# kutieme/avenir

Measured on AMD Instinct MI355X. Metric: naive_bayes_train_rows_per_s, higher is better.
Workload: dtype row-packed categorical records (11-bit records, lossless)/int64 counts (exact); 1 GPU; model=NaiveBayes(resource/churn.json: 5 categorical features, 2 classes), global_batch=1073741824, rows_per_gpu=1073741824, parallelism=dp1

## Files before the change

avenir_amd/csrc/bindings.cpp:

```cpp
#include <algorithm>
#include <atomic>
#include <cstdlib>
#include <condition_variable>
#include <cstring>
#include <functional>
#include <chrono>
#include <limits>
#include <map>
#include <memory>
#include <mutex>
#include <thread>
#include <unistd.h>
#include <sys/stat.h>
#include <sys/mman.h>
#include <fcntl.h>
#include <torch/extension.h>
#include <ATen/hip/impl/HIPGuardImplMasqueradingAsCUDA.h>
#include <ATen/hip/impl/HIPStreamMasqueradingAsCUDA.h>

#include "avenir_kernels.h"
#include "avenir_host.h"

namespace {

// ... 200 lines not shown
                  reinterpret_cast<uint32_t*>(dense.data_ptr<int>()), cur_stream(words));
  return dense;
}

void class_histogram_radix(const at::Tensor& dense, int64_t n, int64_t B, std::vector<int64_t> radices,
                           std::vector<int64_t> bins_host, std::vector<int64_t> offs_host, int64_t class_radix,
                           int64_t total_bins, int64_t n_classes, at::Tensor& out, bool count_labels) {
  CHECK_DEV(dense);
  CHECK_DTYPE(dense, at::kInt);
  TORCH_CHECK(B >= 4 && B <= 15 && n >= 0 && dense.numel() >= avk::dense_words(n, (int)B), "radix stream too short");
  const int64_t F = (int64_t)radices.size();
  TORCH_CHECK(F >= 1 && F <= 8, "1..8 packed fields");
  const auto rad = radix_ints(radices, F, "radices"), hb = radix_ints(bins_host, F, "bins");
  const auto ho = radix_ints(offs_host, F, "offs");
  TORCH_CHECK(n_classes >= 1 && n_classes <= 2, "1 or 2 classes");
  TORCH_CHECK(total_bins >= 1 && total_bins < (int64_t(1) << 24), "bad table width");
  CHECK_DEV(out); CHECK_DTYPE(out, at::kLong);
  TORCH_CHECK(out.numel() == n_classes * total_bins, "out must be [C * TB]");
  DevGuard g(dense.device());
  avk::class_histogram_radix(reinterpret_cast<const uint32_t*>(dense.data_ptr<int>()), n, (int)B, rad.data(), hb.data(),
                             ho.data(), (int)F, (int)class_radix, (int)total_bins, (int)n_classes,
                             count_labels ? 1 : 0, reinterpret_cast<unsigned long long*>(out.data_ptr<int64_t>()),
                             cur_stream(dense));
}

int64_t radix_recip(int64_t d) {
  TORCH_CHECK(d >= 1 && d <= (int64_t(1) << 15), "divisor out of range");
  return (int64_t)avk::radix_recip((unsigned)d);
}

void pair_histogram(const at::Tensor& codes, int64_t n, const c10::optional<at::Tensor>& labels,
                    const at::Tensor& bins, const at::Tensor& pairs, const at::Tensor& poff,
                    int64_t max_tab, int64_t n_classes, at::Tensor& out) {
  CHECK_DEV(codes);
  CHECK_DTYPE(codes, at::kByte);
  TORCH_CHECK(codes.dim() == 2 && n <= codes.size(1), "codes must be [F, ld>=n]");
  CHECK_DEV(bins);
  CHECK_DTYPE(bins, at::kInt);
  CHECK_DEV(pairs);
  CHECK_DTYPE(pairs, at::kInt);
  CHECK_DEV(poff);
  CHECK_DTYPE(poff, at::kLong);
  CHECK_DEV(out);
  CHECK_DTYPE(out, at::kLong);
  TORCH_CHECK(pairs.dim() == 2 && pairs.size(1) == 2, "pairs must be [P,2]");
  TORCH_CHECK(poff.numel() == pairs.size(0), "poff must be [P]");
// ... 4108 lines not shown
  avk::lstm_bwd(dhseq.data_ptr<float>(), reinterpret_cast<const unsigned short*>(gates.data_ptr()),
                cseq.data_ptr<float>(), ptr_or_null<float>(c0), ptr_or_null<float>(dhn), ptr_or_null<float>(dcn),
                wfragT.data_ptr(), (int)B, (int)T, (int)H, (int)KS, RT,
                reinterpret_cast<unsigned short*>(dz.data_ptr()), dh0.data_ptr<float>(), dc0.data_ptr<float>(),
                cur_stream(dhseq));
  return {dz, dh0, dc0};
}

}

void register_comm(py::module_& m);

PYBIND11_MODULE(_C, m) {
  register_comm(m);
  m.doc() = "avenir_amd native kernels (HIP/CDNA4 gfx950) and host runtime";
  m.def("class_histogram", &class_histogram);
  m.def("pair_histogram", &pair_histogram);
  m.def("class_histogram_rowpacked", &class_histogram_rowpacked);
  m.def("pack_dense", &pack_dense);
  m.def("class_histogram_dense", &class_histogram_dense);
  m.def("radix_shape", &radix_shape);
  m.def("pack_radix", &pack_radix);
  m.def("class_histogram_radix", &class_histogram_radix);
  m.def("radix_recip", &radix_recip);
  m.def("bigram_histogram", &bigram_histogram);
  m.def("class_moments", &class_moments);
  m.def("nb_predict", &nb_predict);
  m.def("nb_predict_wide", &nb_predict_wide);
  m.def("node_histogram", &node_histogram, py::arg("codes"), py::arg("n"), py::arg("labels"), py::arg("node"),
        py::arg("weight"), py::arg("bins"), py::arg("offs"), py::arg("total_bins"), py::arg("n_classes"),
        py::arg("n_nodes"), py::arg("hist"), py::arg("node_rows") = py::none());
  m.def("node_grad_histogram", &node_grad_histogram, py::arg("codes"), py::arg("n"), py::arg("node"), py::arg("g"),
        py::arg("h"), py::arg("bins"), py::arg("offs"), py::arg("total_bins"), py::arg("n_nodes"), py::arg("out"),
        py::arg("even_only") = false, py::arg("tot_slot") = -1, py::arg("scale") = 65536.0);
  m.def("gbt_grad", &gbt_grad);
  m.def("gbt_split", &gbt_split);
  m.def("rank_avg", &rank_avg);
  m.def("tfidf_csr", &tfidf_csr);
  m.def("mixed_knn", &mixed_knn);
  m.def("pagerank", &pagerank);
  m.def("pagerank_multi", &pagerank_multi);
  m.def("sgns_hot_replicas", &avk::sgns_hot_replicas);
  m.def("sgns_step", &sgns_step, py::arg("Win"), py::arg("Wout"), py::arg("gIn"), py::arg("gOut"), py::arg("cIn"),
        py::arg("cOut"), py::arg("centre"), py::arg("context"), py::arg("aprob"), py::arg("alias"), py::arg("neg"),
        py::arg("lr"), py::arg("mean_in"), py::arg("seed"), py::arg("step"), py::arg("hot") = py::none(),
        py::arg("gOutHot") = py::none(), py::arg("gInHot") = py::none(), py::arg("cIn_next") = py::none(),
// ... 248 lines not shown
```

avenir_amd/csrc/include/avenir_kernels.h:

```cpp
#pragma once
#include <hip/hip_runtime.h>
#include <stdint.h>
#include <algorithm>
#include <stdexcept>

namespace avk {

void class_histogram(const uint8_t* codes, long long ld, long long n, const uint8_t* labels,
                     const int* d_bins, const int* d_offs, const int* h_bins, int nfeat,
                     int total_bins, int n_classes, int count_labels, unsigned long long* out,
                     int mode, hipStream_t stream);
void class_histogram_wide(const uint16_t* codes, long long ld, long long n, const uint8_t* labels, const int* d_bins,
                          const int* d_offs, int nfeat, int total_bins, int n_classes, int count_labels,
                          unsigned long long* out, int mode, hipStream_t stream);
void class_histogram_i32(const int* codes, long long ld, long long n, const uint8_t* labels, const int* d_bins,
                          const int* d_offs, int nfeat, int total_bins, int n_classes, int count_labels,
                          unsigned long long* out, int mode, hipStream_t stream);
void pair_histogram(const uint8_t* codes, long long ld, long long n, const uint8_t* labels,
                    const int* d_bins, const int* d_pairs, const long long* d_poff, int n_pairs,
                    int max_tab, int n_classes, unsigned long long* out, hipStream_t stream);
void bigram_histogram(const int16_t* states, long long n, int L, const uint8_t* labels,
                      int n_classes, int S, unsigned long long* out, hipStream_t stream);
void class_moments(const float* x, long long ld, long long n, int nfeat, const uint8_t* labels,
                   int n_classes, double* part, int nblocks, double* out, hipStream_t stream);
// ... 297 lines not shown
void linear_act_bwd(const float* dY, const float* Y, float* dZ, float* partial, int M, int N, int act,
                    hipStream_t stream);
int linear_act_wgrad_slices(int M, int N, int K);
void linear_act_wgrad(const float* dY, const float* Y, const float* X, float* dZ, float* pW, float* tmp, float* out,
                      int M, int N, int K, int act, hipStream_t stream);
long long forest_predict_bin_lds(int n_nodes, int nfeat);
void forest_predict_bin(const uint8_t* codes, long long ld, long long n, int nfeat, const uint2* nodes, int n_nodes,
                        const float* values, int V, const int* tree_root, const float* tree_w, int n_trees, int mode,
                        float* out, hipStream_t stream);
long long dense_words(long long n, int B);
void pack_dense(const uint16_t* words, long long n, int B, uint32_t* dense, hipStream_t stream);
void class_histogram_dense(const uint32_t* dense, long long n, int B, const int* h_shift, const int* h_width,
                           int nfeat, int label_shift, int label_width, const int* d_bins, const int* d_offs,
                           int total_bins, int n_classes, int count_labels, unsigned long long* out,
                           hipStream_t stream);
int radix_bits(long long J);
int radix_replicas(long long J, int n_classes, int total_bins);
void pack_radix(const uint16_t* words, long long n, int B, const int* h_shift, const int* h_width, const int* h_radix,
                const int* h_bins, int nfeat, int label_shift, int class_radix, int n_classes, uint32_t* dense,
                hipStream_t stream);
void class_histogram_radix(const uint32_t* dense, long long n, int B, const int* h_radix, const int* h_bins,
                           const int* h_offs, int nfeat, int class_radix, int total_bins, int n_classes,
                           int count_labels, unsigned long long* out, hipStream_t stream);
unsigned radix_recip(unsigned d);
long long csv_chunks(long long size);
unsigned long long csv_slow_tokens_take(hipStream_t stream);
unsigned long long rec_slow_tokens_take(hipStream_t stream);
void csv_newline_counts(const uint8_t* bytes, long long size, unsigned* counts, hipStream_t stream);
void csv_newline_positions(const uint8_t* bytes, long long size, const long long* offsets, long long* pos,
                           hipStream_t stream);
void csv_line_bounds(const uint8_t* bytes, const long long* pos, long long nl, long long* starts, long long* ends,
                     uint8_t* keep, unsigned long long* blank, hipStream_t stream);
void csv_parse_rows(const uint8_t* bytes, long long size_padded, const long long* starts, const long long* ends,
                    long long n, char delim, const void* specs, int nspecs, int max_ord, const int* tabs,
                    const int* voff, const int* vlen, const uint8_t* vbytes, int ntab, int nvoc, int nvb,
                    unsigned long long* short_rows, hipStream_t stream);
int csv_devspec_bytes();
void resample_uniform(unsigned long long seed, unsigned long long stream, long long base, long long n, float* out,
                      hipStream_t st);
void smote(const float* X, const float* Xn, const int* nn, const int* Cs, const int* Cn, long long m, int k, int D,
           int Dc, int mult, long long gbase, unsigned long long seed, int exponential, float exp_mean, float* outX,
           int* outC, int* outPick, hipStream_t st);
void gbt_grad(const float* F, int K, int k, const uint8_t* y, long long n, long long row_off, unsigned long long seed,
              unsigned rate32, float* g, float* h, double* loss, hipStream_t stream);
void gbt_split(const long long* hist, const long long* parent, const long long* left, long long* out_hist, int A,
               int TB, int tot, const int* pfeat, const int* pthr, const int* pstart, const int* pend,
// ... 132 lines not shown
```

avenir_amd/csrc/kernels/histogram.hip:

```cpp
#include <cstdlib>
#include <string>

#include "avenir_common.h"
#include "avenir_kernels.h"

namespace {

constexpr int HB = 256;
constexpr int FLUSH_EVERY = 15;

__device__ __forceinline__ void flush_packed(unsigned long long& lo, unsigned long long& hi,
                                             unsigned int* s_bins ) {
  const unsigned long long M = 0x00FF00FF00FF00FFull;
  unsigned long long w[4] = {lo & M, (lo >> 8) & M, hi & M, (hi >> 8) & M};
#pragma unroll
  for (int q = 0; q < 4; ++q) w[q] = av::wave_sum_u64(w[q]);
  if (av::lane_id() == 0) {
#pragma unroll
    for (int q = 0; q < 4; ++q) {
      const int base = (q >> 1) * 8 + (q & 1);
#pragma unroll
      for (int k = 0; k < 4; ++k) {
        unsigned v = (unsigned)((w[q] >> (16 * k)) & 0xFFFFu);
        if (v) atomicAdd(&s_bins[base + 2 * k], v);
// ... 636 lines not shown
      const int bit = k * B, i = bit >> 5, sh = bit & 31;
#pragma unroll
      for (int q = 0; q < 16; ++q) {
        if (q == i) d[q] |= v << sh;
        if (q == i + 1 && sh + B > 32) d[q] |= v >> (32 - sh);
      }
    }
    for (int i = 0; i < B; ++i) dense[g * B + i] = d[i];
  }
}

struct RadixSpec {
  int rad[8];
  int bins[8];
  int offs[8];
  int crad;
  unsigned stride[8], srcp[8], rrcp[8], crcp;
};

__device__ __forceinline__ unsigned div_small(unsigned n, unsigned d, unsigned m) {
  return d == 1u ? n : __umulhi(n, m);
}

__global__ __launch_bounds__(HB) void pack_radix_kernel(const uint16_t* __restrict__ words, long long n, int B,
                                                        RowPackSpec spec, RadixSpec rs, int nfeat,
                                                        uint32_t* __restrict__ dense) {
  const long long groups = (n + 31) >> 5;
  const long long stride = (long long)gridDim.x * HB;
  for (long long g = (long long)blockIdx.x * HB + threadIdx.x; g < groups; g += stride) {
    uint32_t d[16];
#pragma unroll
    for (int i = 0; i < 16; ++i) d[i] = 0;
    for (int k = 0; k < 32; ++k) {
      const long long r = (g << 5) + k;
      uint32_t v = 0;
      if (r < n) {
        const uint32_t w = words[r];
        uint32_t mult = 1;
        if (rs.crad > 1) {
          const uint32_t lb = __builtin_amdgcn_ubfe(w, (unsigned)spec.lsh, 2u);
          const uint32_t cd = lb == 1u ? 0u : (lb == 2u ? 1u : 2u);
          v = min(cd, (uint32_t)rs.crad - 1u);
          mult = (uint32_t)rs.crad;
        }
        for (int f = 0; f < nfeat; ++f) {
          const uint32_t code = __builtin_amdgcn_ubfe(w, (unsigned)spec.sh[f], (unsigned)spec.w[f]);
          v += min(code, (uint32_t)rs.rad[f] - 1u) * mult;
          mult *= (uint32_t)rs.rad[f];
        }
      }
      const int bit = k * B, i = bit >> 5, sh = bit & 31;
#pragma unroll
      for (int q = 0; q < 16; ++q) {
        if (q == i) d[q] |= v << sh;
        if (q == i + 1 && sh + B > 32) d[q] |= v >> (32 - sh);
      }
    }
    for (int i = 0; i < B; ++i) dense[g * B + i] = d[i];
  }
}

template <int B>
__global__ __launch_bounds__(1024) void hist_joint_radix_kernel(const uint32_t* __restrict__ dense, long long n,
                                                                RadixSpec rs, int J, int log2r, int nfeat,
                                                                int n_classes, int total_bins, int count_labels,
                                                                unsigned long long* __restrict__ out) {
  extern __shared__ __attribute__((aligned(16))) unsigned int s_joint[];
  constexpr unsigned M = (1u << B) - 1u;
  const int NT = (int)blockDim.x;
  const int R = 1 << log2r;
  const int ctb = n_classes * total_bins;
  unsigned int* s_small = s_joint + ((size_t)J << log2r);
  const long long groups = (n + 31) >> 5;
  const long long stride = (long long)gridDim.x * NT;
  uint32_t d[B + 1];
  d[B] = 0;
  auto load = [&](long long g) __attribute__((always_inline)) {
    const uint32_t* src = dense + g * B;
#pragma unroll
    for (int i = 0; i < B; ++i) d[i] = src[i];
  };
  long long g = (long long)blockIdx.x * NT + threadIdx.x;
  if (g < groups) load(g);
  for (int i = threadIdx.x; i < (J << log2r) + ctb; i += NT) s_joint[i] = 0;
  char* const my = reinterpret_cast<char*>(s_joint + (threadIdx.x & (unsigned)(R - 1)));
  const unsigned lr = (unsigned)log2r + 2u;
  __syncthreads();
  while (g < groups) {
    const long long left = n - (g << 5);
    auto rec = [&](int k) __attribute__((always_inline)) -> unsigned {
      const int bit = k * B, i = bit >> 5, sh = bit & 31;
      if (sh + B <= 32) return __builtin_amdgcn_ubfe(d[i], (unsigned)sh, (unsigned)B);
      return __builtin_amdgcn_alignbit(d[i + 1], d[i], (unsigned)sh) & M;
    };
    if (left >= 32) {
#pragma unroll
      for (int k = 0; k < 32; ++k) atomicAdd(reinterpret_cast<unsigned int*>(my + (rec(k) << lr)), 1u);
    } else {
#pragma unroll
      for (int k = 0; k < 32; ++k)
        if (k < left) atomicAdd(reinterpret_cast<unsigned int*>(my + (rec(k) << lr)), 1u);
    }
    g += stride;
    if (g < groups) load(g);
  }
  __syncthreads();
  const int ls = log2r < 3 ? log2r : 3;
  const int S = 1 << ls;
  const int items = J << ls;
  for (int base = 0; base < items; base += NT) {
    const int i = base + (int)threadIdx.x;
    const unsigned cell = (unsigned)(i >> ls);
    unsigned cnt = 0;
    if (i < items)
      for (int q = 0; q < (R >> ls); ++q) cnt += s_joint[((size_t)cell << log2r) + ((i + (q << ls)) & (R - 1))];
    for (int o = S >> 1; o; o >>= 1) cnt += __shfl_xor(cnt, o);
    const unsigned c = cell - div_small(cell, (unsigned)rs.crad, rs.crcp) * (unsigned)rs.crad;
    if (i < items && cnt && c < (unsigned)n_classes) {
      unsigned int* row = s_small + c * total_bins;
      for (int kf = i & (S - 1); kf <= nfeat; kf += S) {
        if (kf == nfeat) {
          if (count_labels) atomicAdd(&row[total_bins - 1], cnt);
          break;
        }
        const unsigned q = div_small(cell, rs.stride[kf], rs.srcp[kf]), rk = (unsigned)rs.rad[kf];
        const unsigned code = q - div_small(q, rk, rs.rrcp[kf]) * rk;
        if (code < (unsigned)rs.bins[kf]) atomicAdd(&row[rs.offs[kf] + code], cnt);
      }
    }
  }
  __syncthreads();
  for (int i = threadIdx.x; i < ctb; i += NT) {
    const unsigned cnt = s_small[i];
    if (cnt) atomicAdd(&out[i], (unsigned long long)cnt);
  }
}

int hist_joint_lds(int nbits, int n_classes, int total_bins) {
  return (int)(sizeof(unsigned) * ((size_t(1) << nbits) + (size_t)n_classes * total_bins));
// ... 472 lines not shown
  if (B < 4 || B > 15 || radix_bits(J) != B) throw std::runtime_error("pack_radix: B = ceil(log2 J) in 4..15");
  RowPackSpec spec{};
  for (int k = 0; k < nfeat; ++k) {
    if (h_width[k] < 1 || h_width[k] > 3 || h_shift[k] < 0 || h_shift[k] + h_width[k] > 16)
      throw std::runtime_error("pack_radix: fields of 1..3 bits inside the 16-bit word");
    spec.sh[k] = h_shift[k];
    spec.w[k] = h_width[k];
  }
  if (n_classes > 1 && (label_shift < 0 || label_shift + 2 > 16))
    throw std::runtime_error("pack_radix: the class is two one-hot bits inside the 16-bit word");
  spec.lsh = n_classes > 1 ? label_shift : 0;
  pack_radix_kernel<<<av::stream_grid((n + 31) >> 5, HB, 1, 4096), HB, 0, stream>>>(words, n, B, spec, rs, nfeat, dense);
  AV_HIP_CHECK(hipGetLastError());
}

int radix_replicas(long long J, int n_classes, int total_bins) {
  int want = 32;
  if (const char* e = std::getenv("AVMI_JOINT_REPLICAS")) want = std::max(1, std::min(32, std::atoi(e)));
  int R = 1;
  while (R * 2 <= want && 4LL * (J * (R * 2) + (long long)n_classes * total_bins) <= kLdsPerCu) R *= 2;
  return R;
}

template <int B>
static void launch_joint_radix(const uint32_t* dense, long long n, const RadixSpec& rs, int J, int nfeat,
                               int n_classes, int total_bins, int count_labels, unsigned long long* out,
                               hipStream_t stream) {
  const int R = radix_replicas(J, n_classes, total_bins);
  const long long lds = 4LL * ((long long)J * R + (long long)n_classes * total_bins);
  if (lds > kLdsPerCu) throw std::runtime_error("radix histogram: joint table exceeds LDS");
  int log2r = 0;
  while ((1 << log2r) < R) ++log2r;
  const int per_cu = (int)(kLdsPerCu / lds);
  const int NT = per_cu >= 4 ? HB : (per_cu >= 2 ? 512 : 1024);
  auto kern = hist_joint_radix_kernel<B>;
  static int c_dev = -1, c_lds = -1, c_nt = 0, c_res = 0;
  int dev = 0;
  AV_HIP_CHECK(hipGetDevice(&dev));
  if (c_dev != dev || c_lds != (int)lds || c_nt != NT) {
    if (lds > 64 * 1024)
      AV_HIP_CHECK(hipFuncSetAttribute(reinterpret_cast<const void*>(kern), hipFuncAttributeMaxDynamicSharedMemorySize,
                                       (int)lds));
    c_res = av::resident_blocks((const void*)kern, NT, (size_t)lds);
    c_dev = dev;
    c_lds = (int)lds;
    c_nt = NT;
  }
  const int grid = std::max(1, std::min(av::stream_grid(std::max(1LL, (n + 31) >> 5), NT, 1, 8192), c_res));
  kern<<<grid, NT, (size_t)lds, stream>>>(dense, n, rs, J, log2r, nfeat, n_classes, total_bins, count_labels, out);
  AV_HIP_CHECK(hipGetLastError());
}

void class_histogram_radix(const uint32_t* dense, long long n, int B, const int* h_radix, const int* h_bins,
                           const int* h_offs, int nfeat, int class_radix, int total_bins, int n_classes,
                           int count_labels, unsigned long long* out, hipStream_t stream) {
  if (n <= 0) return;
  long long J = 0;
  const RadixSpec rs = radix_spec(h_radix, h_bins, h_offs, nfeat, class_radix, n_classes, total_bins, &J);
  if (radix_bits(J) != B) throw std::runtime_error("radix histogram: B = ceil(log2 J)");
  if (count_labels && total_bins < 1) throw std::runtime_error("radix histogram: no class-count column");
  switch (B) {
#define AV_RADIX(BB) \
  case BB: launch_joint_radix<BB>(dense, n, rs, (int)J, nfeat, n_classes, total_bins, count_labels, out, stream); break;
    AV_RADIX(4) AV_RADIX(5) AV_RADIX(6) AV_RADIX(7) AV_RADIX(8) AV_RADIX(9) AV_RADIX(10) AV_RADIX(11)
    AV_RADIX(12) AV_RADIX(13) AV_RADIX(14) AV_RADIX(15)
#undef AV_RADIX
    default: throw std::runtime_error("radix histogram: 4..15 bits per record");
  }
}

}
```

avenir_amd/ops/histogram.py:

```python
from __future__ import annotations

import os

from dataclasses import dataclass
from typing import Sequence

import torch

from .. import _native


_CONST_CACHE: dict = {}


def _dev_i32(vals: Sequence[int], device) -> torch.Tensor:
    key = (tuple(int(v) for v in vals), str(device))
    t = _CONST_CACHE.get(key)
    if t is None:
        if len(_CONST_CACHE) > 4096:
            _CONST_CACHE.clear()
        t = torch.tensor(list(key[0]), dtype=torch.int32, device=device)
        _CONST_CACHE[key] = t
    return t

# ... 30 lines not shown
        idx = lab[ok] * b + v[ok]
        out[:, o:o + b] += torch.bincount(idx, minlength=C * b).view(C, b)
        o += b
    return out


@dataclass
class RowPacked:
    words: torch.Tensor
    n: int
    bins: list[int]
    shifts: list[int]
    widths: list[int]
    label_shift: int
    label_width: int
    n_classes: int
    dense: torch.Tensor | None = None
    bits: int = 16
    radices: list[int] | None = None
    class_radix: int = 1
    dense_is_radix: bool = False
    field_bits: int | None = None
    bitfield: torch.Tensor | None = None

    def ensure_dense(self) -> "RowPacked":
        if self.dense is not None or not self.words.is_cuda or self.n <= 0:
            return self
        if self.radices is not None:
            tb = sum(self.bins) + 1
            _, B, _ = _native.C().radix_shape(list(self.radices), int(self.class_radix), int(self.n_classes), tb)
            if 4 <= B <= 15:
                self.dense = _native.C().pack_radix(self.words, int(self.n), int(B), list(self.shifts),
                                                    list(self.widths), list(self.radices), list(self.bins),
                                                    int(self.label_shift), int(self.class_radix),
                                                    int(self.n_classes))
                self.field_bits, self.bits, self.dense_is_radix = self.bits, int(B), True
                return self
        if 4 <= self.bits <= 15:
            self.dense = _native.C().pack_dense(self.words, int(self.n), int(self.bits))
        return self

    def ensure_bitfield(self) -> torch.Tensor | None:
        if not self.dense_is_radix:
            return self.dense
        if self.bitfield is None and 4 <= self.field_bits <= 15:
            self.bitfield = _native.C().pack_dense(self.words, int(self.n), int(self.field_bits))
        return self.bitfield


def radix_layout(bins: Sequence[int], n_classes: int, missing: Sequence[bool] | None = None,
                 unknown: bool = True, count_labels: bool = True):
    bins = [int(b) for b in bins]
    C = int(n_classes)
    if missing is None:
        missing = [True] * len(bins)
    if not bins or len(bins) > 8 or C < 1 or C > 2 or min(bins) < 1 or max(bins) > 8:
        return None
    radices = [b + 1 if m else b for b, m in zip(bins, missing)]
    class_radix = 1 if C == 1 else (3 if unknown else 2)
    tb = sum(bins) + (1 if count_labels else 0)
    J, B, R = _native.C().radix_shape(radices, class_radix, C, tb)
    if not 4 <= B <= 15:
        return None
    return radices, class_radix, int(J), int(B), int(R)


def rowpack_layout(bins: Sequence[int], n_classes: int, missing: Sequence[bool] | None = None):
    bins = [int(b) for b in bins]
    C = int(n_classes)
    if missing is None:
        missing = [True] * len(bins)
    if not bins or len(bins) > 8 or C < 1 or C > 2 or min(bins) < 1:
        return None
    widths = [max(1, (b if m else b - 1).bit_length()) for b, m in zip(bins, missing)]
    if max(widths) > 3:
        return None
    lw = 2 if C == 2 else 0
    shifts, s = [], lw
    for w in widths:
        shifts.append(s)
        s += w
    if s > 16:
        return None
    return shifts, widths, 0 if lw else s, lw


def pack_rows(codes: torch.Tensor, n: int, bins: Sequence[int], labels: torch.Tensor | None,
# ... 39 lines not shown
        v = (w >> rp.label_shift) & ((1 << rp.label_width) - 1)
        cls = torch.full_like(v, 255)
        for c in range(rp.n_classes):
            cls = torch.where(v == (1 << c), torch.full_like(v, c), cls)
        labels[:n] = cls.to(torch.uint8)
    return codes, labels


def class_histogram_packed(rp: RowPacked, out: torch.Tensor | None = None,
                           count_labels: bool = False) -> torch.Tensor:
    C = rp.n_classes
    tb = sum(rp.bins) + (1 if count_labels else 0)
    if out is None:
        out = torch.zeros((C, tb), dtype=torch.int64, device=rp.words.device)
    if rp.n == 0:
        return out
    if rp.words.is_cuda:
        offs = [0] * len(rp.bins)
        for f in range(1, len(rp.bins)):
            offs[f] = offs[f - 1] + rp.bins[f - 1]
        order = sorted(range(len(rp.bins)), key=lambda k: (C == 2 and rp.widths[k] > 2, k))
        dev = rp.words.device
        kind = os.environ.get("AVMI_ROWPACK_KERNEL", "dense")
        if kind == "dense" and rp.dense_is_radix:
            _native.C().class_histogram_radix(rp.dense, int(rp.n), int(rp.bits), list(rp.radices), list(rp.bins),
                                              offs, int(rp.class_radix), tb, C, out, bool(count_labels))
            return out
        stream = rp.ensure_bitfield() if kind in ("dense", "bitfield") else None
        if stream is not None:
            fb = rp.field_bits if rp.dense_is_radix else rp.bits
            _native.C().class_histogram_dense(stream, int(rp.n), int(fb), list(rp.shifts), list(rp.widths),
                                              rp.label_shift, rp.label_width, _dev_i32(rp.bins, dev),
                                              _dev_i32(offs, dev), tb, C, out, bool(count_labels),
                                              list(rp.bins), offs)
            return out
        _native.C().class_histogram_rowpacked(rp.words, int(rp.n), [rp.shifts[k] for k in order],
                                              [rp.widths[k] for k in order], rp.label_shift, rp.label_width,
                                              _dev_i32([rp.bins[k] for k in order], dev),
                                              _dev_i32([offs[k] for k in order], dev), tb, C, out,
                                              bool(count_labels))
        return out
    codes, labels = unpack_rows(rp)
    return class_histogram(codes, rp.n, rp.bins, labels, C, out=out, count_labels=count_labels)


def pair_histogram(codes: torch.Tensor, n: int, bins: Sequence[int],
                   pairs: Sequence[tuple[int, int]], labels: torch.Tensor | None,
                   n_classes: int) -> list[torch.Tensor]:
    bins = [int(b) for b in bins]
    C = int(n_classes) if labels is not None else 1
    sizes = [C * bins[a] * bins[b] for a, b in pairs]
# ... 63 lines not shown
```

Measured before the change: 4212 billion rows/s.

## Add frequency-ranked patched bit stream with exception list for radix histogram

Joint radix states are ranked by frequency from a row sample. Records are re-encoded into a narrower b-bit stream in which the most frequent states get short codes, and rare states store an escape code plus a separate sorted exception list. The histogram kernel gains a patched variant that counts an extra escape cell and then adds the exception cells back. The aim is to cut the bytes read by a bandwidth-bound histogram, at the cost of an extra packing pass, data-dependent sizing, and extra atomic work for the exceptions.

```diff
diff --git a/avenir_amd/csrc/bindings.cpp b/avenir_amd/csrc/bindings.cpp
--- a/avenir_amd/csrc/bindings.cpp
+++ b/avenir_amd/csrc/bindings.cpp
@@ -246,6 +246,110 @@
                              ho.data(), (int)F, (int)class_radix, (int)total_bins, (int)n_classes,
                              count_labels ? 1 : 0, reinterpret_cast<unsigned long long*>(out.data_ptr<int64_t>()),
                              cur_stream(dense));
+}
+
+static int64_t patched_states(int64_t b, const std::vector<int64_t>& radices, int64_t class_radix) {
+  TORCH_CHECK(b >= 4 && b <= 14, "patched stream: 4..14 bits per record");
+  TORCH_CHECK(class_radix >= 1 && class_radix <= 3, "bad class radix");
+  int64_t J = class_radix;
+  for (int64_t r : radices) {
+    TORCH_CHECK(r >= 1 && r <= 9, "radix out of range");
+    J *= r;
+    TORCH_CHECK(J + 1 <= (int64_t(1) << 15), "patched stream: more than 2^15 cells");
+  }
+  TORCH_CHECK((int64_t(1) << b) < J, "patched stream: b must be below ceil(log2 J)");
+  return J;
+}
+
+std::tuple<at::Tensor, at::Tensor> pack_patched(const at::Tensor& words, int64_t n, int64_t b,
+                                                std::vector<int64_t> shifts, std::vector<int64_t> widths,
+                                                std::vector<int64_t> radices, std::vector<int64_t> bins_host,
+                                                int64_t label_shift, int64_t class_radix, int64_t n_classes,
+                                                const at::Tensor& state_cell) {
+  CHECK_DEV(words);
+  CHECK_DTYPE(words, at::kShort);
+  TORCH_CHECK(words.dim() == 1 && n >= 0 && n <= words.numel(), "words must be [>= n]");
+  const int64_t F = (int64_t)shifts.size();
+  TORCH_CHECK(F >= 1 && F <= 8, "1..8 packed fields");
+  const auto sh = radix_ints(shifts, F, "shifts"), wd = radix_ints(widths, F, "widths");
+  const auto rad = radix_ints(radices, F, "radices"), hb = radix_ints(bins_host, F, "bins");
+  const int64_t J = patched_states(b, radices, class_radix);
+  CHECK_DEV(state_cell);
+  CHECK_DTYPE(state_cell, at::kShort);
+  TORCH_CHECK(state_cell.is_contiguous() && state_cell.numel() == J && state_cell.device() == words.device(),
+              "state_cell must be [J] on the words' device");
+  auto dense = at::zeros({std::max<int64_t>(1, avk::dense_words(n, (int)b))}, words.options().dtype(at::kInt));
+  auto n_exc = at::zeros({1}, words.options().dtype(at::kLong));
+  DevGuard g(words.device());
+  avk::pack_patched(reinterpret_cast<const uint16_t*>(words.data_ptr()), n, (int)b, sh.data(), wd.data(), rad.data(),
+                    hb.data(), (int)F, (int)label_shift, (int)class_radix, (int)n_classes,
+                    reinterpret_cast<const uint16_t*>(state_cell.data_ptr()),
+                    reinterpret_cast<uint32_t*>(dense.data_ptr<int>()),
+                    reinterpret_cast<unsigned long long*>(n_exc.data_ptr<int64_t>()), cur_stream(words));
+  return {dense, n_exc};
+}
+
+std::tuple<at::Tensor, at::Tensor> patch_exceptions(const at::Tensor& words, int64_t n, int64_t b,
+                                                    std::vector<int64_t> shifts, std::vector<int64_t> widths,
+                                                    std::vector<int64_t> radices, std::vector<int64_t> bins_host,
+                                                    int64_t label_shift, int64_t class_radix, int64_t n_classes,
+                                                    const at::Tensor& state_cell, int64_t n_exc) {
+  CHECK_DEV(words);
+  CHECK_DTYPE(words, at::kShort);
+  TORCH_CHECK(words.dim() == 1 && n >= 0 && n <= words.numel(), "words must be [>= n]");
+  TORCH_CHECK(n_exc >= 0 && n_exc <= n, "0 <= escaped records <= n");
+  const int64_t F = (int64_t)shifts.size();
+  TORCH_CHECK(F >= 1 && F <= 8, "1..8 packed fields");
+  const auto sh = radix_ints(shifts, F, "shifts"), wd = radix_ints(widths, F, "widths");
+  const auto rad = radix_ints(radices, F, "radices"), hb = radix_ints(bins_host, F, "bins");
+  const int64_t J = patched_states(b, radices, class_radix);
+  CHECK_DEV(state_cell);
+  CHECK_DTYPE(state_cell, at::kShort);
+  TORCH_CHECK(state_cell.is_contiguous() && state_cell.numel() == J && state_cell.device() == words.device(),
+              "state_cell must be [J] on the words' device");
+  auto idx = at::zeros({n_exc}, words.options().dtype(at::kLong));
+  auto cell = at::zeros({n_exc}, words.options().dtype(at::kShort));
+  auto fill = at::zeros({1}, words.options().dtype(at::kLong));
+  DevGuard g(words.device());
+  avk::patch_exceptions(reinterpret_cast<const uint16_t*>(words.data_ptr()), n, (int)b, sh.data(), wd.data(),
+                        rad.data(), hb.data(), (int)F, (int)label_shift, (int)class_radix, (int)n_classes,
+                        reinterpret_cast<const uint16_t*>(state_cell.data_ptr()), n_exc,
+                        reinterpret_cast<long long*>(idx.data_ptr<int64_t>()),
+                        reinterpret_cast<uint16_t*>(cell.data_ptr()),
+                        reinterpret_cast<unsigned long long*>(fill.data_ptr<int64_t>()), cur_stream(words));
+  return {idx, cell};
+}
+
+void class_histogram_patched(const at::Tensor& dense, int64_t n, int64_t b, std::vector<int64_t> radices,
+                             std::vector<int64_t> bins_host, std::vector<int64_t> offs_host, int64_t class_radix,
+                             int64_t total_bins, int64_t n_classes, at::Tensor& out, bool count_labels,
+                             const at::Tensor& exc_cell, const at::Tensor& cell_state) {
+  CHECK_DEV(dense);
+  CHECK_DTYPE(dense, at::kInt);
+  const int64_t J = patched_states(b, radices, class_radix);
+  TORCH_CHECK(n >= 0 && dense.is_contiguous() && dense.numel() >= avk::dense_words(n, (int)b),
+              "patched stream too short");
+  const int64_t F = (int64_t)radices.size();
+  TORCH_CHECK(F >= 1 && F <= 8, "1..8 packed fields");
+  const auto rad = radix_ints(radices, F, "radices"), hb = radix_ints(bins_host, F, "bins");
+  const auto ho = radix_ints(offs_host, F, "offs");
+  TORCH_CHECK(n_classes >= 1 && n_classes <= 2, "1 or 2 classes");
+  TORCH_CHECK(total_bins >= 1 && total_bins < (int64_t(1) << 24), "bad table width");
+  CHECK_DEV(exc_cell); CHECK_DTYPE(exc_cell, at::kShort);
+  CHECK_DEV(cell_state); CHECK_DTYPE(cell_state, at::kShort);
+  TORCH_CHECK(exc_cell.dim() == 1 && exc_cell.is_contiguous() && exc_cell.numel() <= n &&
+                  exc_cell.device() == dense.device(), "exc_cell must be [E <= n] on the stream's device");
+  TORCH_CHECK(reinterpret_cast<uintptr_t>(exc_cell.data_ptr()) % 16 == 0, "exc_cell must be 16-byte aligned");
+  TORCH_CHECK(cell_state.is_contiguous() && cell_state.numel() == J + 1 && cell_state.device() == dense.device(),
+              "cell_state must be [J + 1] on the stream's device");
+  CHECK_DEV(out); CHECK_DTYPE(out, at::kLong);
+  TORCH_CHECK(out.numel() == n_classes * total_bins && out.device() == dense.device(), "out must be [C * TB]");
+  DevGuard g(dense.device());
+  avk::class_histogram_patched(reinterpret_cast<const uint32_t*>(dense.data_ptr<int>()), n, (int)b, rad.data(),
+                               hb.data(), ho.data(), (int)F, (int)class_radix, (int)total_bins, (int)n_classes,
+                               count_labels ? 1 : 0, reinterpret_cast<const uint16_t*>(exc_cell.data_ptr()),
+                               exc_cell.numel(), reinterpret_cast<const uint16_t*>(cell_state.data_ptr()),
+                               reinterpret_cast<unsigned long long*>(out.data_ptr<int64_t>()), cur_stream(dense));
 }
 
 int64_t radix_recip(int64_t d) {
@@ -4400,6 +4504,9 @@
   m.def("radix_shape", &radix_shape);
   m.def("pack_radix", &pack_radix);
   m.def("class_histogram_radix", &class_histogram_radix);
+  m.def("pack_patched", &pack_patched);
+  m.def("patch_exceptions", &patch_exceptions);
+  m.def("class_histogram_patched", &class_histogram_patched);
   m.def("radix_recip", &radix_recip);
   m.def("bigram_histogram", &bigram_histogram);
   m.def("class_moments", &class_moments);
diff --git a/avenir_amd/csrc/include/avenir_kernels.h b/avenir_amd/csrc/include/avenir_kernels.h
--- a/avenir_amd/csrc/include/avenir_kernels.h
+++ b/avenir_amd/csrc/include/avenir_kernels.h
@@ -343,6 +343,17 @@
 void class_histogram_radix(const uint32_t* dense, long long n, int B, const int* h_radix, const int* h_bins,
                            const int* h_offs, int nfeat, int class_radix, int total_bins, int n_classes,
                            int count_labels, unsigned long long* out, hipStream_t stream);
+void pack_patched(const uint16_t* words, long long n, int b, const int* h_shift, const int* h_width,
+                  const int* h_radix, const int* h_bins, int nfeat, int label_shift, int class_radix, int n_classes,
+                  const uint16_t* state_cell, uint32_t* dense, unsigned long long* n_exc, hipStream_t stream);
+void patch_exceptions(const uint16_t* words, long long n, int b, const int* h_shift, const int* h_width,
+                      const int* h_radix, const int* h_bins, int nfeat, int label_shift, int class_radix,
+                      int n_classes, const uint16_t* state_cell, long long n_exc, long long* exc_index,
+                      uint16_t* exc_cell, unsigned long long* fill, hipStream_t stream);
+void class_histogram_patched(const uint32_t* dense, long long n, int b, const int* h_radix, const int* h_bins,
+                             const int* h_offs, int nfeat, int class_radix, int total_bins, int n_classes,
+                             int count_labels, const uint16_t* exc_cell, long long n_exc, const uint16_t* cell_state,
+                             unsigned long long* out, hipStream_t stream);
 unsigned radix_recip(unsigned d);
 long long csv_chunks(long long size);
 unsigned long long csv_slow_tokens_take(hipStream_t stream);
diff --git a/avenir_amd/csrc/kernels/histogram.hip b/avenir_amd/csrc/kernels/histogram.hip
--- a/avenir_amd/csrc/kernels/histogram.hip
+++ b/avenir_amd/csrc/kernels/histogram.hip
@@ -682,6 +682,22 @@
   return d == 1u ? n : __umulhi(n, m);
 }
 
+__device__ __forceinline__ uint32_t radix_code(uint32_t w, const RowPackSpec& spec, const RadixSpec& rs, int nfeat) {
+  uint32_t v = 0, mult = 1;
+  if (rs.crad > 1) {
+    const uint32_t lb = __builtin_amdgcn_ubfe(w, (unsigned)spec.lsh, 2u);
+    const uint32_t cd = lb == 1u ? 0u : (lb == 2u ? 1u : 2u);
+    v = min(cd, (uint32_t)rs.crad - 1u);
+    mult = (uint32_t)rs.crad;
+  }
+  for (int f = 0; f < nfeat; ++f) {
+    const uint32_t code = __builtin_amdgcn_ubfe(w, (unsigned)spec.sh[f], (unsigned)spec.w[f]);
+    v += min(code, (uint32_t)rs.rad[f] - 1u) * mult;
+    mult *= (uint32_t)rs.rad[f];
+  }
+  return v;
+}
+
 __global__ __launch_bounds__(HB) void pack_radix_kernel(const uint16_t* __restrict__ words, long long n, int B,
                                                         RowPackSpec spec, RadixSpec rs, int nfeat,
                                                         uint32_t* __restrict__ dense) {
@@ -693,22 +709,7 @@
     for (int i = 0; i < 16; ++i) d[i] = 0;
     for (int k = 0; k < 32; ++k) {
       const long long r = (g << 5) + k;
-      uint32_t v = 0;
-      if (r < n) {
-        const uint32_t w = words[r];
-        uint32_t mult = 1;
-        if (rs.crad > 1) {
-          const uint32_t lb = __builtin_amdgcn_ubfe(w, (unsigned)spec.lsh, 2u);
-          const uint32_t cd = lb == 1u ? 0u : (lb == 2u ? 1u : 2u);
-          v = min(cd, (uint32_t)rs.crad - 1u);
-          mult = (uint32_t)rs.crad;
-        }
-        for (int f = 0; f < nfeat; ++f) {
-          const uint32_t code = __builtin_amdgcn_ubfe(w, (unsigned)spec.sh[f], (unsigned)spec.w[f]);
-          v += min(code, (uint32_t)rs.rad[f] - 1u) * mult;
-          mult *= (uint32_t)rs.rad[f];
-        }
-      }
+      const uint32_t v = r < n ? radix_code(words[r], spec, rs, nfeat) : 0u;
       const int bit = k * B, i = bit >> 5, sh = bit & 31;
 #pragma unroll
       for (int q = 0; q < 16; ++q) {
@@ -720,17 +721,91 @@
   }
 }
 
-template <int B>
+__device__ __forceinline__ uint32_t patched_cell(uint32_t w, const RowPackSpec& spec, const RadixSpec& rs, int nfeat,
+                                                 const uint16_t* s_cell) {
+  return s_cell[radix_code(w, spec, rs, nfeat)];
+}
+
+__global__ __launch_bounds__(HB) void pack_patched_kernel(const uint16_t* __restrict__ words, long long n, int b,
+                                                          RowPackSpec spec, RadixSpec rs, int J, int nfeat,
+                                                          const uint16_t* __restrict__ state_cell,
+                                                          uint32_t* __restrict__ dense,
+                                                          unsigned long long* __restrict__ n_exc) {
+  extern __shared__ __attribute__((aligned(16))) uint16_t s_cell[];
+  for (int i = threadIdx.x; i < J; i += HB) s_cell[i] = state_cell[i];
+  __syncthreads();
+  const uint32_t esc = (1u << b) - 1u;
+  const long long groups = (n + 31) >> 5;
+  const long long stride = (long long)gridDim.x * HB;
+  unsigned long long mine = 0;
+  for (long long g = (long long)blockIdx.x * HB + threadIdx.x; g < groups; g += stride) {
+    uint32_t d[16];
+#pragma unroll
+    for (int i = 0; i < 16; ++i) d[i] = 0;
+    for (int k = 0; k < 32; ++k) {
+      const long long r = (g << 5) + k;
+      uint32_t v = 0;
+      if (r < n) {
+        v = patched_cell(words[r], spec, rs, nfeat, s_cell);
+        if (v > esc) {
+          v = esc;
+          ++mine;
+        }
+      }
+      const int bit = k * b, i = bit >> 5, sh = bit & 31;
+#pragma unroll
+      for (int q = 0; q < 16; ++q) {
+        if (q == i) d[q] |= v << sh;
+        if (q == i + 1 && sh + b > 32) d[q] |= v >> (32 - sh);
+      }
+    }
+    for (int i = 0; i < b; ++i) dense[g * b + i] = d[i];
+  }
+  if (mine) atomicAdd(n_exc, mine);
+}
+
+__global__ __launch_bounds__(HB) void patch_exceptions_kernel(const uint16_t* __restrict__ words, long long n, int b,
+                                                              RowPackSpec spec, RadixSpec rs, int J, int nfeat,
+                                                              const uint16_t* __restrict__ state_cell,
+                                                              long long* __restrict__ exc_index,
+                                                              uint16_t* __restrict__ exc_cell,
+                                                              unsigned long long* __restrict__ fill,
+                                                              unsigned long long cap) {
+  extern __shared__ __attribute__((aligned(16))) uint16_t s_cell[];
+  for (int i = threadIdx.x; i < J; i += HB) s_cell[i] = state_cell[i];
+  __syncthreads();
+  const uint32_t esc = (1u << b) - 1u;
+  const long long stride = (long long)gridDim.x * HB;
+  for (long long r = (long long)blockIdx.x * HB + threadIdx.x; r < n; r += stride) {
+    const uint32_t v = patched_cell(words[r], spec, rs, nfeat, s_cell);
+    if (v > esc) {
+      const unsigned long long at = atomicAdd(fill, 1ull);
+      if (at < cap) {
+        exc_index[at] = r;
+        exc_cell[at] = (uint16_t)v;
+      }
+    }
+  }
+}
+
+struct PatchSpec {
+  const uint16_t* exc_cell;
+  const uint16_t* cell_state;
+  long long n_exc;
+};
+
+template <int B, bool P>
 __global__ __launch_bounds__(1024) void hist_joint_radix_kernel(const uint32_t* __restrict__ dense, long long n,
                                                                 RadixSpec rs, int J, int log2r, int nfeat,
                                                                 int n_classes, int total_bins, int count_labels,
-                                                                unsigned long long* __restrict__ out) {
+                                                                unsigned long long* __restrict__ out, PatchSpec ps) {
   extern __shared__ __attribute__((aligned(16))) unsigned int s_joint[];
   constexpr unsigned M = (1u << B) - 1u;
   const int NT = (int)blockDim.x;
   const int R = 1 << log2r;
   const int ctb = n_classes * total_bins;
-  unsigned int* s_small = s_joint + ((size_t)J << log2r);
+  const int cells = P ? J + 1 : J;
+  unsigned int* s_small = s_joint + ((size_t)cells << log2r);
   const long long groups = (n + 31) >> 5;
   const long long stride = (long long)gridDim.x * NT;
   uint32_t d[B + 1];
@@ -742,7 +817,7 @@
   };
   long long g = (long long)blockIdx.x * NT + threadIdx.x;
   if (g < groups) load(g);
-  for (int i = threadIdx.x; i < (J << log2r) + ctb; i += NT) s_joint[i] = 0;
+  for (int i = threadIdx.x; i < (cells << log2r) + ctb; i += NT) s_joint[i] = 0;
   char* const my = reinterpret_cast<char*>(s_joint + (threadIdx.x & (unsigned)(R - 1)));
   const unsigned lr = (unsigned)log2r + 2u;
   __syncthreads();
@@ -764,17 +839,40 @@
     g += stride;
     if (g < groups) load(g);
   }
+  if (P) {
+    auto add = [&](unsigned c) __attribute__((always_inline)) {
+      atomicAdd(reinterpret_cast<unsigned int*>(my + (min(c, (unsigned)J) << lr)), 1u);
+    };
+    const long long octs = ps.n_exc >> 3;
+    const uint4* src = reinterpret_cast<const uint4*>(ps.exc_cell);
+    const long long first = (long long)blockIdx.x * NT + threadIdx.x;
+    for (long long e = first; e < octs; e += stride) {
+      const uint4 v = src[e];
+      const unsigned w[4] = {v.x, v.y, v.z, v.w};
+#pragma unroll
+      for (int k = 0; k < 4; ++k) {
+        add(w[k] & 0xFFFFu);
+        add(w[k] >> 16);
+      }
+    }
+    for (long long e = (octs << 3) + first; e < ps.n_exc; e += stride) add(ps.exc_cell[e]);
+  }
   __syncthreads();
   const int ls = log2r < 3 ? log2r : 3;
   const int S = 1 << ls;
-  const int items = J << ls;
+  const int items = cells << ls;
   for (int base = 0; base < items; base += NT) {
     const int i = base + (int)threadIdx.x;
-    const unsigned cell = (unsigned)(i >> ls);
+    const unsigned slot = (unsigned)(i >> ls);
     unsigned cnt = 0;
     if (i < items)
-      for (int q = 0; q < (R >> ls); ++q) cnt += s_joint[((size_t)cell << log2r) + ((i + (q << ls)) & (R - 1))];
+      for (int q = 0; q < (R >> ls); ++q) cnt += s_joint[((size_t)slot << log2r) + ((i + (q << ls)) & (R - 1))];
     for (int o = S >> 1; o; o >>= 1) cnt += __shfl_xor(cnt, o);
+    unsigned cell = slot;
+    if (P) {
+      cell = i < items && slot != M ? (unsigned)ps.cell_state[slot] : (unsigned)J;
+      if (cell >= (unsigned)J) cnt = 0;
+    }
     const unsigned c = cell - div_small(cell, (unsigned)rs.crad, rs.crcp) * (unsigned)rs.crad;
     if (i < items && cnt && c < (unsigned)n_classes) {
       unsigned int* row = s_small + c * total_bins;
@@ -1293,18 +1391,19 @@
   return R;
 }
 
-template <int B>
+template <int B, bool P>
 static void launch_joint_radix(const uint32_t* dense, long long n, const RadixSpec& rs, int J, int nfeat,
                                int n_classes, int total_bins, int count_labels, unsigned long long* out,
-                               hipStream_t stream) {
-  const int R = radix_replicas(J, n_classes, total_bins);
-  const long long lds = 4LL * ((long long)J * R + (long long)n_classes * total_bins);
+                               const PatchSpec& ps, hipStream_t stream) {
+  const int cells = P ? J + 1 : J;
+  const int R = radix_replicas(cells, n_classes, total_bins);
+  const long long lds = 4LL * ((long long)cells * R + (long long)n_classes * total_bins);
   if (lds > kLdsPerCu) throw std::runtime_error("radix histogram: joint table exceeds LDS");
   int log2r = 0;
   while ((1 << log2r) < R) ++log2r;
   const int per_cu = (int)(kLdsPerCu / lds);
   const int NT = per_cu >= 4 ? HB : (per_cu >= 2 ? 512 : 1024);
-  auto kern = hist_joint_radix_kernel<B>;
+  auto kern = hist_joint_radix_kernel<B, P>;
   static int c_dev = -1, c_lds = -1, c_nt = 0, c_res = 0;
   int dev = 0;
   AV_HIP_CHECK(hipGetDevice(&dev));
@@ -1318,7 +1417,8 @@
     c_nt = NT;
   }
   const int grid = std::max(1, std::min(av::stream_grid(std::max(1LL, (n + 31) >> 5), NT, 1, 8192), c_res));
-  kern<<<grid, NT, (size_t)lds, stream>>>(dense, n, rs, J, log2r, nfeat, n_classes, total_bins, count_labels, out);
+  kern<<<grid, NT, (size_t)lds, stream>>>(dense, n, rs, J, log2r, nfeat, n_classes, total_bins, count_labels, out,
+                                          ps);
   AV_HIP_CHECK(hipGetLastError());
 }
 
@@ -1332,7 +1432,10 @@
   if (count_labels && total_bins < 1) throw std::runtime_error("radix histogram: no class-count column");
   switch (B) {
 #define AV_RADIX(BB) \
-  case BB: launch_joint_radix<BB>(dense, n, rs, (int)J, nfeat, n_classes, total_bins, count_labels, out, stream); break;
+  case BB:                                                                                                  \
+    launch_joint_radix<BB, false>(dense, n, rs, (int)J, nfeat, n_classes, total_bins, count_labels, out, PatchSpec{}, \
+                                  stream);                                                                  \
+    break;
     AV_RADIX(4) AV_RADIX(5) AV_RADIX(6) AV_RADIX(7) AV_RADIX(8) AV_RADIX(9) AV_RADIX(10) AV_RADIX(11)
     AV_RADIX(12) AV_RADIX(13) AV_RADIX(14) AV_RADIX(15)
 #undef AV_RADIX
@@ -1340,4 +1443,76 @@
   }
 }
 
-}
+static void patched_check(long long J, int b) {
+  if (b < 4 || b > 14 || b >= radix_bits(J)) throw std::runtime_error("patched stream: 4 <= b < ceil(log2 J), b <= 14");
+  if (J + 1 > (1LL << 15)) throw std::runtime_error("patched stream: more than 2^15 cells");
+}
+
+static RowPackSpec patched_fields(const int* h_shift, const int* h_width, int nfeat, int label_shift, int n_classes) {
+  RowPackSpec spec{};
+  for (int k = 0; k < nfeat; ++k) {
+    if (h_width[k] < 1 || h_width[k] > 3 || h_shift[k] < 0 || h_shift[k] + h_width[k] > 16)
+      throw std::runtime_error("patched stream: fields of 1..3 bits inside the 16-bit word");
+    spec.sh[k] = h_shift[k];
+    spec.w[k] = h_width[k];
+  }
+  if (n_classes > 1 && (label_shift < 0 || label_shift + 2 > 16))
+    throw std::runtime_error("patched stream: the class is two one-hot bits inside the 16-bit word");
+  spec.lsh = n_classes > 1 ? label_shift : 0;
+  return spec;
+}
+
+void pack_patched(const uint16_t* words, long long n, int b, const int* h_shift, const int* h_width,
+                  const int* h_radix, const int* h_bins, int nfeat, int label_shift, int class_radix, int n_classes,
+                  const uint16_t* state_cell, uint32_t* dense, unsigned long long* n_exc, hipStream_t stream) {
+  if (n <= 0) return;
+  const int offs0[8] = {0, 0, 0, 0, 0, 0, 0, 0};
+  long long J = 0;
+  const RadixSpec rs = radix_spec(h_radix, h_bins, offs0, nfeat, class_radix, n_classes, 1 << 30, &J);
+  patched_check(J, b);
+  const RowPackSpec spec = patched_fields(h_shift, h_width, nfeat, label_shift, n_classes);
+  pack_patched_kernel<<<av::stream_grid((n + 31) >> 5, HB, 1, 4096), HB, (size_t)J * sizeof(uint16_t), stream>>>(
+      words, n, b, spec, rs, (int)J, nfeat, state_cell, dense, n_exc);
+  AV_HIP_CHECK(hipGetLastError());
+}
+
+void patch_exceptions(const uint16_t* words, long long n, int b, const int* h_shift, const int* h_width,
+                      const int* h_radix, const int* h_bins, int nfeat, int label_shift, int class_radix,
+                      int n_classes, const uint16_t* state_cell, long long n_exc, long long* exc_index,
+                      uint16_t* exc_cell, unsigned long long* fill, hipStream_t stream) {
+  if (n <= 0 || n_exc <= 0) return;
+  const int offs0[8] = {0, 0, 0, 0, 0, 0, 0, 0};
+  long long J = 0;
+  const RadixSpec rs = radix_spec(h_radix, h_bins, offs0, nfeat, class_radix, n_classes, 1 << 30, &J);
+  patched_check(J, b);
+  const RowPackSpec spec = patched_fields(h_shift, h_width, nfeat, label_shift, n_classes);
+  patch_exceptions_kernel<<<av::stream_grid(n, HB, 1, 4096), HB, (size_t)J * sizeof(uint16_t), stream>>>(
+      words, n, b, spec, rs, (int)J, nfeat, state_cell, exc_index, exc_cell, fill, (unsigned long long)n_exc);
+  AV_HIP_CHECK(hipGetLastError());
+}
+
+void class_histogram_patched(const uint32_t* dense, long long n, int b, const int* h_radix, const int* h_bins,
+                             const int* h_offs, int nfeat, int class_radix, int total_bins, int n_classes,
+                             int count_labels, const uint16_t* exc_cell, long long n_exc, const uint16_t* cell_state,
+                             unsigned long long* out, hipStream_t stream) {
+  if (n <= 0) return;
+  long long J = 0;
+  const RadixSpec rs = radix_spec(h_radix, h_bins, h_offs, nfeat, class_radix, n_classes, total_bins, &J);
+  patched_check(J, b);
+  if (n_exc < 0 || (n_exc > 0 && !exc_cell) || (reinterpret_cast<uintptr_t>(exc_cell) & 15u) || !cell_state)
+    throw std::runtime_error("patched histogram: exception list (16-byte aligned) and cell table");
+  if (count_labels && total_bins < 1) throw std::runtime_error("patched histogram: no class-count column");
+  const PatchSpec ps{exc_cell, cell_state, n_exc};
+  switch (b) {
+#define AV_PATCHED(BB)                                                                                          \
+  case BB:                                                                                                      \
+    launch_joint_radix<BB, true>(dense, n, rs, (int)J, nfeat, n_classes, total_bins, count_labels, out, ps, stream); \
+    break;
+    AV_PATCHED(4) AV_PATCHED(5) AV_PATCHED(6) AV_PATCHED(7) AV_PATCHED(8) AV_PATCHED(9) AV_PATCHED(10) AV_PATCHED(11)
+    AV_PATCHED(12) AV_PATCHED(13) AV_PATCHED(14)
+#undef AV_PATCHED
+    default: throw std::runtime_error("patched histogram: 4..14 bits per record");
+  }
+}
+
+}
diff --git a/avenir_amd/ops/histogram.py b/avenir_amd/ops/histogram.py
--- a/avenir_amd/ops/histogram.py
+++ b/avenir_amd/ops/histogram.py
@@ -76,6 +76,12 @@
     dense_is_radix: bool = False
     field_bits: int | None = None
     bitfield: torch.Tensor | None = None
+    patched: torch.Tensor | None = None
+    patched_bits: int | None = None
+    exc_index: torch.Tensor | None = None
+    exc_cell: torch.Tensor | None = None
+    cell_state: torch.Tensor | None = None
+    state_cell: torch.Tensor | None = None
 
     def ensure_dense(self) -> "RowPacked":
         if self.dense is not None or not self.words.is_cuda or self.n <= 0:
@@ -89,6 +95,7 @@
                                                     int(self.label_shift), int(self.class_radix),
                                                     int(self.n_classes))
                 self.field_bits, self.bits, self.dense_is_radix = self.bits, int(B), True
+                attach_patched(self)
                 return self
         if 4 <= self.bits <= 15:
             self.dense = _native.C().pack_dense(self.words, int(self.n), int(self.bits))
@@ -117,6 +124,149 @@
     if not 4 <= B <= 15:
         return None
     return radices, class_radix, int(J), int(B), int(R)
+
+
+PATCH_SAMPLE = 1 << 20
+PATCH_MARGIN = 0.937
+
+
+def patch_ranks(counts) -> torch.Tensor:
+    c = torch.as_tensor(counts, dtype=torch.int64).cpu()
+    order = torch.sort(-c, stable=True).indices
+    rank = torch.empty_like(order)
+    rank[order] = torch.arange(c.numel())
+    return rank
+
+
+def patch_tables(counts, b: int) -> tuple[torch.Tensor, torch.Tensor]:
+    rank = patch_ranks(counts)
+    J, esc = rank.numel(), (1 << int(b)) - 1
+    if not 4 <= int(b) <= 14 or esc + 1 >= J or J + 1 > 1 << 15:
+        raise ValueError("patched stream: 4 <= b < ceil(log2 J), b <= 14, J + 1 <= 2^15")
+    state_cell = torch.where(rank < esc, rank, rank + 1)
+    cell_state = torch.full((J + 1,), -1, dtype=torch.int64)
+    cell_state[state_cell] = torch.arange(J)
+    return state_cell.to(torch.int16), cell_state.to(torch.int16)
+
+
+def patch_cost(counts, b: int) -> float:
+    c = torch.as_tensor(counts, dtype=torch.int64).cpu()
+    top = torch.sort(c, descending=True).values
+    return b / 8.0 + 2.0 * float(top[(1 << b) - 1:].sum()) / max(1, int(c.sum()))
+
+
+def choose_patch_bits(counts, margin: float = PATCH_MARGIN) -> int | None:
+    J = int(torch.as_tensor(counts).numel())
+    B = max(0, J - 1).bit_length()
+    if J + 1 > 1 << 15 or int(torch.as_tensor(counts).sum()) <= 0:
+        return None
+    best = None
+    for b in range(4, min(B, 15)):
+        cost = patch_cost(counts, b)
+        if best is None or cost < best[0]:
+            best = (cost, b)
+    if best is None or not best[0] < margin * B / 8.0:
+        return None
+    return best[1]
+
+
+def patch_keep(b: int, B: int, n: int, n_exc: int, margin: float = PATCH_MARGIN) -> bool:
+    groups = (int(n) + 31) // 32
+    return b * groups * 4 + 2 * int(n_exc) < margin * (B * groups * 4)
+
+
+def _pack_bits(v: torch.Tensor, B: int) -> torch.Tensor:
+    v = v.long().cpu()
+    n = v.numel()
+    r = torch.arange(n)
+    pos = (r // 32) * (32 * B) + (r % 32) * B
+    acc = torch.zeros((n + 31) // 32 * B, dtype=torch.int64)
+    for i in range(B):
+        acc.index_add_(0, (pos + i) // 32, ((v >> i) & 1) << ((pos + i) % 32))
+    return torch.where(acc >= 1 << 31, acc - (1 << 32), acc).to(torch.int32)
+
+
+def _unpack_bits(dense: torch.Tensor, n: int, B: int) -> torch.Tensor:
+    d = dense.long().cpu() & 0xFFFFFFFF
+    r = torch.arange(n)
+    pos = (r // 32) * (32 * B) + (r % 32) * B
+    v = torch.zeros(n, dtype=torch.int64)
+    for i in range(B):
+        v |= ((d[(pos + i) // 32] >> ((pos + i) % 32)) & 1) << i
+    return v
+
+
+def ref_patch_encode(code: torch.Tensor, state_cell: torch.Tensor, b: int):
+    cell = state_cell.long().cpu()[code.long().cpu()]
+    esc = (1 << int(b)) - 1
+    out = cell > esc
+    stream = _pack_bits(torch.where(out, torch.full_like(cell, esc), cell), int(b))
+    return stream, out.nonzero().flatten(), cell[out].to(torch.int16)
+
+
+def ref_patch_decode(stream: torch.Tensor, n: int, b: int, exc_index: torch.Tensor, exc_cell: torch.Tensor,
+                     cell_state: torch.Tensor) -> torch.Tensor:
+    cell = _unpack_bits(stream, int(n), int(b))
+    esc = (1 << int(b)) - 1
+    idx = exc_index.long().cpu()
+    assert torch.equal((cell == esc).nonzero().flatten(), idx), "the exceptions are the records that store ESC"
+    cell[idx] = exc_cell.long().cpu() & 0xFFFF
+    return cell_state.long().cpu()[cell]
+
+
+def _radix_codes(rp: "RowPacked", words: torch.Tensor) -> torch.Tensor:
+    w = words.to(torch.int64) & 0xFFFF
+    code = torch.zeros_like(w)
+    mult = 1
+    if rp.class_radix > 1:
+        lb = (w >> rp.label_shift) & 3
+        cd = torch.where(lb == 1, torch.zeros_like(lb), torch.where(lb == 2, torch.ones_like(lb), torch.full_like(lb, 2)))
+        code = cd.clamp_max(rp.class_radix - 1)
+        mult = rp.class_radix
+    for s, wd, r in zip(rp.shifts, rp.widths, rp.radices):
+        code = code + ((w >> s) & ((1 << wd) - 1)).clamp_max(r - 1) * mult
+        mult *= r
+    return code
+
+
+def attach_patched(rp: "RowPacked", bits: int | None = None, sample: torch.Tensor | None = None,
+                   margin: float | None = None) -> "RowPacked":
+    rp.patched = rp.patched_bits = rp.exc_index = rp.exc_cell = rp.cell_state = rp.state_cell = None
+    if not rp.dense_is_radix or not rp.words.is_cuda or rp.n <= 0:
+        return rp
+    margin = PATCH_MARGIN if margin is None else float(margin)
+    J = int(rp.class_radix)
+    for r in rp.radices:
+        J *= int(r)
+    B = int(rp.bits)
+    if B < 5 or J + 1 > 1 << 15:
+        return rp
+    picked = rp.words[:rp.n:-(-rp.n // PATCH_SAMPLE)] if sample is None else rp.words[sample]
+    counts = torch.bincount(_radix_codes(rp, picked), minlength=J).cpu()
+    if bits is None:
+        b = choose_patch_bits(counts, margin)
+        if b is None:
+            return rp
+    else:
+        b = int(bits)
+        if not 4 <= b < B:
+            raise ValueError("patched stream: 4 <= bits < ceil(log2 J)")
+    state_cell, cell_state = patch_tables(counts, b)
+    dev = rp.words.device
+    state_cell, cell_state = state_cell.to(dev), cell_state.to(dev)
+    lay = (int(rp.n), b, list(rp.shifts), list(rp.widths), list(rp.radices), list(rp.bins), int(rp.label_shift),
+           int(rp.class_radix), int(rp.n_classes), state_cell)
+    stream, n_exc = _native.C().pack_patched(rp.words, *lay)
+    E = int(n_exc.item())
+    if bits is None and not patch_keep(b, B, rp.n, E, margin):
+        return rp
+    idx, cell = _native.C().patch_exceptions(rp.words, *lay, E)
+    if E:
+        idx, order = torch.sort(idx)
+        cell = cell[order]
+    rp.patched, rp.patched_bits, rp.exc_index, rp.exc_cell = stream, b, idx, cell
+    rp.cell_state, rp.state_cell = cell_state, state_cell
+    return rp
 
 
 def rowpack_layout(bins: Sequence[int], n_classes: int, missing: Sequence[bool] | None = None):
@@ -202,11 +352,16 @@
         order = sorted(range(len(rp.bins)), key=lambda k: (C == 2 and rp.widths[k] > 2, k))
         dev = rp.words.device
         kind = os.environ.get("AVMI_ROWPACK_KERNEL", "dense")
-        if kind == "dense" and rp.dense_is_radix:
+        if kind == "dense" and rp.patched is not None:
+            _native.C().class_histogram_patched(rp.patched, int(rp.n), int(rp.patched_bits), list(rp.radices),
+                                                list(rp.bins), offs, int(rp.class_radix), tb, C, out,
+                                                bool(count_labels), rp.exc_cell, rp.cell_state)
+            return out
+        if kind in ("dense", "radix") and rp.dense_is_radix:
             _native.C().class_histogram_radix(rp.dense, int(rp.n), int(rp.bits), list(rp.radices), list(rp.bins),
                                               offs, int(rp.class_radix), tb, C, out, bool(count_labels))
             return out
-        stream = rp.ensure_bitfield() if kind in ("dense", "bitfield") else None
+        stream = rp.ensure_bitfield() if kind in ("dense", "radix", "bitfield") else None
         if stream is not None:
             fb = rp.field_bits if rp.dense_is_radix else rp.bits
             _native.C().class_histogram_dense(stream, int(rp.n), int(fb), list(rp.shifts), list(rp.widths),
```

Measured after the change: 4616 billion rows/s, median of 6. 1.1x the previous value.
